# mjevans26/Satellite_ComputerVision

Measured on AMD Instinct MI355X. Metric: tiles/sec (train) 256x256x4 U-Net, higher is better.
Workload: dtype bf16; 1 GPU; U-Net 256x256x4 bfloat16 training, batch 64 per GPU (BASELINE configs[1]); global_batch=64, parallelism=dp1, loss=weighted_categorical_crossentropy, optimizer=adam(9e-4)

## Files before the change

satellite_computervision_amd/csrc/conv_bwd_fused.hip:

```cpp
#include "igemm_common.hpp"
#include <cstdlib>
#include <cstring>

#ifndef BWDF_ABL
#define BWDF_ABL 0
#endif
#define FABL(bit) ((BWDF_ABL & (bit)) != 0)

int wgrad_reduce_slabs(const float* ws, float* dw, int nslab, int taps, int kpad, int npad, int cin, int nvalid, int accumulate, hipStream_t st);
void reduce_job_fill(satcv_reduce_job* job, const float* ws, float* dw, int nslab, int taps, int kpad, int npad, int cin, int nvalid, int transposed, int accumulate);
void satcv_prof_begin(int kind, double flops, hipStream_t st);
void satcv_prof_end(int kind, hipStream_t st);

struct BwdfArgs {
  IgemmArgs e;
  const void* g; const void* yraw; int ldg;
  const float* bn_scale; const float* bn_shift; const float* bn_mean; const float* bn_rstd; const float* bn_coef; int bn_c, linear;
  const void* x0; const void* x1; int c0, c1;
  const float* in_scale; const float* in_shift; int in_relu;
  const void* w;
  float* ws;
  int tiles_x, tiles_y;
  satcv_stat_t* bst_sums; int bst_ld; const float* bst_mean; const float* bst_rstd;
  int bst_act_form;
  const void* dp; int lddp; const unsigned char* amax;
  const float* hg_dl; const float* hg_w;
};

__device__ __forceinline__ bf16x4 tr_read4(const bf16* p) {
  short4v v = __builtin_amdgcn_ds_read_tr16_b64_v4i16((__attribute__((address_space(3))) short4v*)(p));
  return __builtin_bit_cast(bf16x4, v);
}

template <int CIN, int COUT, int NW, int WPS, bool POOL = false, bool NODG = false, int CINS = CIN, bool HG = false>
__global__ __launch_bounds__(NW * 64, WPS) void bwd_fused_kernel(const BwdfArgs a, const int total_tiles) {
  static_assert(!HG || !POOL, "the head feeds a decoder block");
  typedef bf16 T;
  constexpr int TW = 32, TH = 8, BM = 256, RL = TH + 2, CL = TW + 2, PITCH = CL, EL = 8, NTHREADS = NW * 64;
  constexpr int SD = COUT / 8, SX = CIN / 8, SXR = CINS / 8;
  constexpr int DSTRIDE = RL * PITCH * EL;
  constexpr int XSTRIDE = BM * EL + 32;
  static_assert((DSTRIDE * 2) % 256 == 64 && (XSTRIDE * 2) % 256 == 64, "plane strides must be 64 B modulo 256 B");
  constexpr int D_ITEMS = RL * CL * SD, DI = (D_ITEMS + NTHREADS - 1) / NTHREADS;
  constexpr int X_ITEMS = BM * SXR, XI = X_ITEMS / NTHREADS;
  static_assert(X_ITEMS % NTHREADS == 0 && NTHREADS % SD == 0 && NTHREADS % SXR == 0, "item -> thread mapping");
  constexpr int XPIX_STEP = NTHREADS / SXR;
  static_assert(XPIX_STEP % 32 == 0, "x items of a thread must share a column");
  constexpr int MT = 8 / NW, NT = CIN / 32;
#ifdef BWDF_NOBAL
  constexpr int NTILE = (CIN / 32) * (COUT / 32) * 9, FULL = (NTILE + NW - 1) / NW, REM = 0, WT = FULL;
#else
  constexpr int NTILE = (CIN / 32) * (COUT / 32) * 9, FULL = NTILE / NW, REM = NTILE % NW, WT = FULL + (REM ? 1 : 0);
#endif
  constexpr bool GUARD = FULL * NW > NTILE;
  constexpr int WPP = REM ? NW / REM : 1, KPW = REM ? 16 / WPP : 0;
  static_assert(REM == 0 || (NW % REM == 0 && 16 % WPP == 0 && KPW % 2 == 0), "left-over products must split evenly along K");
  constexpr int W_ITEMS = NODG ? 0 : 9 * SD * CIN;
  constexpr size_t R0_BYTES = ((size_t)(SD * DSTRIDE + SX * XSTRIDE) * sizeof(T) + 127) / 128 * 128;
  constexpr size_t W_BYTES = (size_t)W_ITEMS * EL * sizeof(T);
  constexpr size_t O_BYTES = (size_t)BM * (CIN + 8) * sizeof(T);
  constexpr bool O_ALIAS = O_BYTES <= (size_t)SD * DSTRIDE * sizeof(T);
  constexpr size_t TAB_BYTES = (size_t)(SD * 32 + SX * 16 + (HG ? 2 * COUT : 0)) * sizeof(float);
  static_assert(!NODG || O_ALIAS || true, "");
  constexpr size_t O_OFF = O_ALIAS ? 0 : (R0_BYTES + W_BYTES + TAB_BYTES + 127) / 128 * 128;
  extern __shared__ __attribute__((aligned(16))) unsigned char smem_raw[];
  T* ldsD = reinterpret_cast<T*>(smem_raw);
  T* ldsX = ldsD + SD * DSTRIDE;
  T* ldsW = reinterpret_cast<T*>(smem_raw + R0_BYTES);
  float* tabD = reinterpret_cast<float*>(smem_raw + R0_BYTES + W_BYTES);
  float* tabX = tabD + SD * 32;
  float* tabH = tabX + SX * 16;

  const int tid = threadIdx.x, lane = tid & 63, wave = tid >> 6;
  const int r = lane & 31, hh = lane >> 5;
  const T* wp = reinterpret_cast<const T*>(a.w);

  for (int it = tid; it < W_ITEMS; it += NTHREADS) lstore8<T>(ldsW + (size_t)it * EL, gload8<T>(wp + (size_t)it * EL));
  if constexpr (SXR < SX) {
    for (int it = tid; it < (SX - SXR) * BM; it += NTHREADS) lstore8<T>(ldsX + (SXR + it / BM) * XSTRIDE + (it % BM) * EL, zero8<T>());
  }
  for (int ch = tid; ch < COUT; ch += NTHREADS) {
    const float sc = a.bn_scale[ch], sh = a.bn_shift[ch], mu = a.bn_mean[ch], rs = a.bn_rstd[ch], c1 = a.bn_coef[ch], c2 = a.bn_coef[a.bn_c + ch];
    float* t = tabD + (ch >> 3) * 32 + (ch & 7);
    t[0] = sc; t[8] = sh; t[16] = -sc * c2 * rs; t[24] = sc * (c2 * rs * mu - c1);
  }
  if constexpr (HG) {
    for (int ch = tid; ch < COUT; ch += NTHREADS) {
      float* t = tabH + (ch >> 3) * 16 + (ch & 7);
      t[0] = a.hg_w[ch * 2]; t[8] = a.hg_w[ch * 2 + 1];
    }
  }
  for (int ch = tid; ch < CINS; ch += NTHREADS) {
    float* t = tabX + (ch >> 3) * 16 + (ch & 7);
    t[0] = a.in_scale ? a.in_scale[ch] : 1.f; t[8] = a.in_scale ? a.in_shift[ch] : 0.f;
  }
  const float lin_lo = a.linear ? -INFINITY : 0.f;
  const bool xaff = a.in_scale != nullptr;
  const unsigned xrelu_lim = a.in_relu != 0 ? 0u : 0x80008000u;

  const int slot_d = tid % SD, slot_x = tid % SXR;
  constexpr int DPK = (DI + 2) / 3;
  unsigned d_pk[DPK];
#pragma unroll
  for (int k = 0; k < DPK; ++k) d_pk[k] = 0;
#pragma unroll
  for (int j = 0; j < DI; ++j) {
    const int it = tid + j * NTHREADS;
    const int p = it / SD, c = p % CL, L = p / CL;
    d_pk[j / 3] |= (unsigned)(it < D_ITEMS ? (L << 6) | c : 0x3ff) << (10 * (j % 3));
  }
  auto d_item = [&](int j) -> int { return (int)((d_pk[j / 3] >> (10 * (j % 3))) & 0x3ffu); };
  const int g_rowstride = a.e.w_ * a.ldg;
  const unsigned gy_lane = (unsigned)slot_d * EL;
  const int xch0 = slot_x * EL;
  const bool xsecond = xch0 >= a.c0;
  const T* xsrc = xsecond ? reinterpret_cast<const T*>(a.x1) + (xch0 - a.c0) : reinterpret_cast<const T*>(a.x0) + xch0;
  const int xcs = xsecond ? a.c1 : a.c0;
  const int xq0 = tid / SXR;
  const int x_l0 = slot_x * XSTRIDE + xq0 * EL;
  const int x_eoff0 = ((xq0 / TW) * a.e.w_ + (xq0 % TW)) * xcs, x_estep = (XPIX_STEP / TW) * a.e.w_ * xcs;

  int a_off[MT];
#pragma unroll
  for (int m = 0; m < MT; ++m) {
    const int q = (wave * MT + m) * 32 + r;
    a_off[m] = ((q / TW) * PITCH + (q % TW)) * EL;
  }
  const int gi = lane >> 4, i16 = lane & 15;
  const int chb = 16 * (gi & 1) + 4 * (i16 & 3);
  const int pk = 8 * (gi >> 1) + (i16 >> 2);
  const int tr_x = (chb >> 3) * XSTRIDE + pk * EL + (chb & 7);
  const int tr_d = (chb >> 3) * DSTRIDE + pk * EL + (chb & 7);

  auto tile_origin = [&](int v, int& n0, int& y0, int& x0) {
    const int tx = v % a.tiles_x; v /= a.tiles_x;
    const int ty = v % a.tiles_y;
    n0 = v / a.tiles_y; y0 = ty * TH; x0 = tx * TW;
  };
  auto next_origin = [&](int& n0, int& y0, int& x0) {
    x0 += TW;
    if (x0 >= a.e.w_) { x0 = 0; y0 += TH; if (y0 >= a.e.h) { y0 = 0; ++n0; } }
  };
  Raw8<T> rg[HG ? 1 : DI], ry[DI], rx[XI];
  float2 rdl[HG ? DI : 1];
  Raw8<T> rp[POOL ? DI : 1];
  uint2 ra[POOL ? DI : 1];
  const int hp = a.e.h >> 1, wpool = a.e.w_ >> 1;
  unsigned valid = 0;
  auto issue_loads = [&](int n0, int y0, int x0) -> unsigned {
    unsigned vm = 0;
    const int ylo = 1 - y0, yhi = a.e.h - y0 + 1, xlo = 1 - x0, xhi = a.e.w_ - x0 + 1;
    const long long pb = (long long)(n0 * a.e.h + y0 - 1) * a.e.w_ + (x0 - 1);
    const long long bp = pb * a.ldg;
    const T* gb = reinterpret_cast<const T*>(a.g) + bp;
    const T* yb = reinterpret_cast<const T*>(a.yraw) + bp;
    const unsigned centre = (unsigned)(g_rowstride + a.ldg) + gy_lane;
#pragma unroll
    for (int j = 0; j < DI; ++j) {
      const int pk_ = d_item(j), L = pk_ >> 6, c = pk_ & 63;
      const bool ok = pk_ != 0x3ff && L >= ylo && L < yhi && c >= xlo && c < xhi;
      vm |= (ok ? 1u : 0u) << j;
      unsigned off = ok ? (unsigned)(__mul24(L, g_rowstride) + __mul24(c, a.ldg)) + gy_lane : centre;
      asm volatile("" : "+v"(off));
      if constexpr (HG) {
        int poff = ok ? __mul24(L, a.e.w_) + c : a.e.w_ + 1;
        asm volatile("" : "+v"(poff));
        rdl[j] = reinterpret_cast<const float2*>(a.hg_dl)[pb + poff];
        ry[j] = gload8<T>(yb + off);
      } else if (!FABL(32)) { rg[j] = gload8<T>(gb + off); ry[j] = gload8<T>(yb + off); }
      else { rg[j] = zero8<T>(); ry[j] = zero8<T>(); rg[j].q[0].x = off; }
    }
    return vm;
  };
  auto issue_pool = [&](int n0, int y0, int x0) {
    if constexpr (POOL) {
      const int ylo = 1 - y0, yhi = a.e.h - y0 + 1, xlo = 1 - x0, xhi = a.e.w_ - x0 + 1;
      const size_t pb = (size_t)(n0 * hp + (y0 >> 1)) * wpool + (x0 >> 1);
#pragma unroll
      for (int j = 0; j < DI; ++j) {
        const int pk_ = d_item(j), L = pk_ >> 6, c = pk_ & 63;
        const bool ok = pk_ != 0x3ff && L >= ylo && L < yhi && c >= xlo && c < xhi;
        int po = ok ? __mul24((L - 1) >> 1, wpool) + ((c - 1) >> 1) : 0;
        asm volatile("" : "+v"(po));
        rp[j] = gload8<T>(reinterpret_cast<const T*>(a.dp) + (pb + po) * a.lddp + gy_lane);
        ra[j] = *reinterpret_cast<const uint2*>(a.amax + (pb + po) * COUT + gy_lane);
      }
    }
  };
  auto issue_x = [&](int n0, int y0, int x0) {
    const size_t bp = (size_t)(n0 * a.e.h + y0) * a.e.w_ + x0;
    const T* xb = xsrc + bp * xcs + x_eoff0;
#pragma unroll
    for (int j = 0; j < XI; ++j) { if (!FABL(32)) rx[j] = gload8<T>(xb + (size_t)j * x_estep); else { rx[j] = zero8<T>(); rx[j].q[0].x = (unsigned)(size_t)xb; } }
  };

  const int G = gridDim.x;
  const int xcd = blockIdx.x & 7, nx = G >> 3, remx = G & 7;
  const int bid = (xcd < remx ? xcd * (nx + 1) : remx * (nx + 1) + (xcd - remx) * nx) + (blockIdx.x >> 3);
  const int per = total_tiles / G, extra = total_tiles % G;
  const int t_lo = bid * per + (bid < extra ? bid : extra), t_hi = t_lo + per + (bid < extra ? 1 : 0);

  f32x16 wacc[WT];
  int w_xo[WT], w_do[WT];
#pragma unroll
  for (int t = 0; t < WT; ++t) {
#pragma unroll
    for (int i = 0; i < 16; ++i) wacc[t][i] = 0.f;
    const int wv = __builtin_amdgcn_readfirstlane(wave);
    const int id = t < FULL ? wv + t * NW : FULL * NW + wv / WPP;
    const int tap = id % 9, pair = id / 9;
    const int ci_t = pair % (CIN / 32), co_t = pair / (CIN / 32);
    w_xo[t] = ci_t * 4 * XSTRIDE;
    w_do[t] = co_t * 4 * DSTRIDE + ((2 - tap / 3) * PITCH + (2 - tap % 3)) * EL;
    if (t >= FULL) {
      const int k0 = (wv % WPP) * KPW;
      w_xo[t] += k0 * 16 * EL;
      w_do[t] += (k0 >> 1) * PITCH * EL;
    }
  }

  constexpr bool BST = !NODG && (WPS != 1 || POOL);
  float bs1[8], bs2[8];
#pragma unroll
  for (int e = 0; e < 8; ++e) { bs1[e] = 0.f; bs2[e] = 0.f; }
  int n0, y0, x0;
  if (t_lo < t_hi) { tile_origin(t_lo, n0, y0, x0); valid = issue_loads(n0, y0, x0); issue_x(n0, y0, x0); issue_pool(n0, y0, x0); }
  __syncthreads();
  for (int t = t_lo; t < t_hi; ++t) {
    {
      int toff = slot_d * 32;
      asm volatile("" : "+v"(toff));
      const float4* tp = reinterpret_cast<const float4*>(tabD + toff);
      float prm[32];
#pragma unroll
      for (int k = 0; k < 8; ++k) { const float4 v4 = tp[k]; prm[4 * k] = v4.x; prm[4 * k + 1] = v4.y; prm[4 * k + 2] = v4.z; prm[4 * k + 3] = v4.w; }
#pragma unroll
      for (int j = 0; j < DI; ++j) {
        float gv[8], yv[8];
        if constexpr (HG) {
          int hoff = slot_d * 16;
          asm volatile("" : "+v"(hoff));
          const float4* hp = reinterpret_cast<const float4*>(tabH + hoff);
          const float4 w00 = hp[0], w01 = hp[1], w10 = hp[2], w11 = hp[3];
          const float w0[8] = {w00.x, w00.y, w00.z, w00.w, w01.x, w01.y, w01.z, w01.w};
          const float w1[8] = {w10.x, w10.y, w10.z, w10.w, w11.x, w11.y, w11.z, w11.w};
#pragma unroll
          for (int e = 0; e < 8; ++e) gv[e] = (float)(T)fmaf(rdl[j].y, w1[e], rdl[j].x * w0[e]);
        } else {
          unpack8<T>(rg[j], gv);
        }
        unpack8<T>(ry[j], yv);
        if constexpr (POOL) {
          float pv[8];
          unpack8<T>(rp[j], pv);
          const int pk2 = d_item(j);
          const unsigned sub = ((((pk2 >> 6) + 1) & 1) << 1) | (((pk2 & 63) + 1) & 1);
#pragma unroll
          for (int e = 0; e < 8; ++e) {
            const unsigned am = ((e < 4 ? ra[j].x : ra[j].y) >> (8 * (e & 3))) & 0xffu;
            gv[e] += am == sub ? pv[e] : 0.f;
          }
        }
        Raw8<T> v;
        if constexpr (FABL(2) && !HG) { v = rg[j]; v.q[0].x ^= ry[j].q[0].x; }
        else {
          bf16x8 o;
#pragma unroll
          for (int e = 0; e < 8; ++e) {
            const float act = yv[e] * prm[e] + prm[8 + e];
            const float gm = act > lin_lo ? gv[e] : 0.f;
            o[e] = (bf16)(prm[e] * gm + (prm[16 + e] * yv[e] + prm[24 + e]));
          }
          v.q[0] = __builtin_bit_cast(uint4, o);
        }
        v = select8<T>((valid >> j) & 1u, v);
        const int pk_ = d_item(j);
        if (pk_ != 0x3ff) lstore8<T>(ldsD + slot_d * DSTRIDE + __mul24((pk_ >> 6) * CL + (pk_ & 63), EL), v);
        __builtin_amdgcn_sched_barrier(0);
      }
    }
    {
      float sc[8], sh[8];
      if (xaff) {
        int toff = slot_x * 16;
        asm volatile("" : "+v"(toff));
        const float4* tp = reinterpret_cast<const float4*>(tabX + toff);
        const float4 s0 = tp[0], s1 = tp[1], h0 = tp[2], h1 = tp[3];
        sc[0] = s0.x; sc[1] = s0.y; sc[2] = s0.z; sc[3] = s0.w; sc[4] = s1.x; sc[5] = s1.y; sc[6] = s1.z; sc[7] = s1.w;
        sh[0] = h0.x; sh[1] = h0.y; sh[2] = h0.z; sh[3] = h0.w; sh[4] = h1.x; sh[5] = h1.y; sh[6] = h1.z; sh[7] = h1.w;
      }
#pragma unroll
      for (int j = 0; j < XI; ++j) {
        Raw8<T> v = rx[j];
        if (xaff) v = affine8_lim(v, sc, sh, xrelu_lim);
        lstore8<T>(ldsX + x_l0 + j * (XPIX_STEP * EL), v);
      }
    }
    __syncthreads();
    const int tn0 = n0, ty0 = y0, tx0 = x0;
    if (t + 1 < t_hi) { next_origin(n0, y0, x0); valid = issue_loads(n0, y0, x0); }

#pragma unroll
    for (int tt = 0; tt < FULL; ++tt) {
      if (!FABL(8) && (!GUARD || tt < FULL - 1 || __builtin_amdgcn_readfirstlane(wave) + (FULL - 1) * NW < NTILE)) {
        const T* xa = ldsX + w_xo[tt] + tr_x;
        const T* da = ldsD + w_do[tt] + tr_d;
        bf16x4 fa[2][2], fb[2][2];
        auto read_k = [&](const T* xp, const T* dp, int u, int buf) {
          const int xq = u * 16 * EL, dq = ((u >> 1) * PITCH + (u & 1) * 16) * EL;
          fa[buf][0] = tr_read4(xp + xq); fa[buf][1] = tr_read4(xp + xq + 4 * EL);
          fb[buf][0] = tr_read4(dp + dq); fb[buf][1] = tr_read4(dp + dq + 4 * EL);
        };
        read_k(xa, da, 0, 0);
#pragma unroll 1
        for (int grp = 0; grp < TH / 2; ++grp) {
          const T* xp = xa + grp * (64 * EL);
          const T* dp = da + grp * (2 * PITCH * EL);
          const int wrap = grp + 1 < TH / 2 ? 1 : 1 - TH / 2;
#pragma unroll
          for (int u = 0; u < 4; ++u) {
            asm volatile("" ::: "memory");
            if (u < 3) read_k(xp, dp, u + 1, (u + 1) & 1);
            else read_k(xp + wrap * (64 * EL), dp + wrap * (2 * PITCH * EL), 0, 0);
            __builtin_amdgcn_sched_barrier(0);
            const bf16x8 afr = __builtin_shufflevector(fa[u & 1][0], fa[u & 1][1], 0, 1, 2, 3, 4, 5, 6, 7);
            const bf16x8 bfr = __builtin_shufflevector(fb[u & 1][0], fb[u & 1][1], 0, 1, 2, 3, 4, 5, 6, 7);
            if constexpr (!FABL(1)) wacc[tt] = __builtin_amdgcn_mfma_f32_32x32x16_bf16(afr, bfr, wacc[tt], 0, 0, 0);
            else asm volatile("" :: "v"(afr), "v"(bfr));
          }
        }
      }
    }
    if constexpr (REM > 0) {
      if (!FABL(8)) {
        const T* xa = ldsX + w_xo[FULL] + tr_x;
        const T* da = ldsD + w_do[FULL] + tr_d;
        bf16x4 fa[2][2], fb[2][2];
        auto read_k = [&](int u, int buf) {
          const int xq = u * 16 * EL, dq = ((u >> 1) * PITCH + (u & 1) * 16) * EL;
          fa[buf][0] = tr_read4(xa + xq); fa[buf][1] = tr_read4(xa + xq + 4 * EL);
          fb[buf][0] = tr_read4(da + dq); fb[buf][1] = tr_read4(da + dq + 4 * EL);
        };
        read_k(0, 0);
#pragma unroll
        for (int u = 0; u < KPW; ++u) {
          asm volatile("" ::: "memory");
          if (u + 1 < KPW) read_k(u + 1, (u + 1) & 1);
          __builtin_amdgcn_sched_barrier(0);
          const bf16x8 afr = __builtin_shufflevector(fa[u & 1][0], fa[u & 1][1], 0, 1, 2, 3, 4, 5, 6, 7);
          const bf16x8 bfr = __builtin_shufflevector(fb[u & 1][0], fb[u & 1][1], 0, 1, 2, 3, 4, 5, 6, 7);
          if constexpr (!FABL(1)) wacc[FULL] = __builtin_amdgcn_mfma_f32_32x32x16_bf16(afr, bfr, wacc[FULL], 0, 0, 0);
          else asm volatile("" :: "v"(afr), "v"(bfr));
        }
      }
    }
    if (t + 1 < t_hi) issue_x(n0, y0, x0);
    if (POOL && NODG && t + 1 < t_hi) issue_pool(n0, y0, x0);
    if constexpr (!NODG) {
    f32x16 acc[MT][NT];
#pragma unroll
    for (int m = 0; m < MT; ++m)
#pragma unroll
      for (int n = 0; n < NT; ++n)
#pragma unroll
        for (int i = 0; i < 16; ++i) acc[m][n][i] = 0.f;
    {
      constexpr int KS = COUT / 16, STEPS = 9 * KS;
      FragT<T> af[2][MT], bf[2][NT];
      auto read_step = [&](int st, int buf) {
        const int tap = st / KS, ks = st % KS;
        const int tap_off = ((tap / 3) * PITCH + (tap % 3)) * EL;
        const int slot = ks * 2 + hh;
#pragma unroll
        for (int m = 0; m < MT; ++m) af[buf][m] = lds_frag<T>(ldsD + slot * DSTRIDE + a_off[m] + tap_off);
#pragma unroll
        for (int n = 0; n < NT; ++n) bf[buf][n] = lds_frag<T>(ldsW + ((tap * SD + slot) * CIN + n * 32 + r) * EL);
      };
      if constexpr (!FABL(8)) {
      read_step(0, 0);
#pragma unroll
      for (int st = 0; st < STEPS; ++st) {
        asm volatile("" ::: "memory");
        if (st + 1 < STEPS) read_step(st + 1, (st + 1) & 1);
        __builtin_amdgcn_sched_barrier(0);
#pragma unroll
        for (int m = 0; m < MT; ++m)
#pragma unroll
          for (int n = 0; n < NT; ++n) {
            if constexpr (!FABL(1)) mma32<T>(acc[m][n], af[st & 1][m], bf[st & 1][n]);
            else asm volatile("" :: "v"(af[st & 1][m].v), "v"(bf[st & 1][n].v));
          }
      }
      }
    }
    if (POOL && t + 1 < t_hi) issue_pool(n0, y0, x0);
    __syncthreads();
    {
      constexpr int OPITCH = CIN + 8, VPR = CIN / 8;
      T* ldsO = reinterpret_cast<T*>(smem_raw + O_OFF);
      T* op = ldsO + ((wave * MT) * 32 + 4 * hh) * OPITCH + r;
#pragma unroll
      for (int m = 0; m < MT; ++m)
#pragma unroll
        for (int n = 0; n < NT; ++n)
#pragma unroll
          for (int i = 0; i < 16; ++i) op[(m * 32 + (i & 3) + 8 * (i >> 2)) * OPITCH + n * 32] = (T)acc[m][n][i];
      __syncthreads();
      const int vq = tid % VPR;
      T* yp = reinterpret_cast<T*>(a.e.y) + ((size_t)(tn0 * a.e.h + ty0) * a.e.w_ + tx0) * a.e.ldy + vq * 8;
      const unsigned row_pitch = (unsigned)a.e.w_ * a.e.ldy;
      const T* xact = ldsX + vq * XSTRIDE;
#pragma unroll 2
      for (int it = tid; it < BM * VPR; it += NTHREADS) {
        const int q = it / VPR;
        const uint4 dv = *reinterpret_cast<const uint4*>(ldsO + q * OPITCH + vq * 8);
        if constexpr (!FABL(4)) *reinterpret_cast<uint4*>(yp + (size_t)((q / TW) * row_pitch + (q % TW) * (unsigned)a.e.ldy)) = dv;
        else asm volatile("" :: "v"(dv.x));
        if (BST && a.bst_sums) {
          const bf16x8 d8 = __builtin_bit_cast(bf16x8, dv);
          const bf16x8 a8 = *reinterpret_cast<const bf16x8*>(xact + q * EL);
#pragma unroll
          for (int e = 0; e < 8; ++e) {
            const float df = (float)d8[e], af = (float)a8[e];
            bs1[e] += af > 0.f ? df : 0.f;
            bs2[e] += df * af;
          }
        }
      }
    }
    }
    __syncthreads();
  }
  if constexpr (REM > 0) {
    float* red = reinterpret_cast<float*>(smem_raw);
#pragma unroll
    for (int i = 0; i < 16; ++i) red[(wave * 16 + i) * 64 + lane] = wacc[FULL][i];
    __syncthreads();
    if (wave % WPP == 0) {
#pragma unroll 1
      for (int k = 1; k < WPP; ++k)
#pragma unroll
        for (int i = 0; i < 16; ++i) wacc[FULL][i] += red[((wave + k) * 16 + i) * 64 + lane];
    }
  }
#pragma unroll
  for (int tt = 0; tt < WT; ++tt) {
    const int wv = __builtin_amdgcn_readfirstlane(wave);
    const int id = tt < FULL ? wv + tt * NW : FULL * NW + wv / WPP;
    if ((tt < FULL && (!GUARD || id < NTILE)) || (tt >= FULL && wv % WPP == 0)) {
      const int tap = id % 9, pair = id / 9;
      const int ci_t = pair % (CIN / 32), co_t = pair / (CIN / 32);
      float* dst = a.ws + ((size_t)(blockIdx.x * 9 + tap) * CIN + ci_t * 32) * COUT + co_t * 32 + r;
#pragma unroll
      for (int i = 0; i < 16; ++i) dst[(size_t)((i & 3) + 8 * (i >> 2) + 4 * hh) * COUT] = wacc[tt][i];
    }
  }
  if (BST && a.bst_sums && t_lo < t_hi) {
    constexpr int VPR = CIN / 8, NPER = NTHREADS / VPR;
    float* red = reinterpret_cast<float*>(smem_raw);
    __syncthreads();
#pragma unroll
    for (int e = 0; e < 8; ++e) { red[e * NTHREADS + tid] = bs1[e]; red[(8 + e) * NTHREADS + tid] = bs2[e]; }
    __syncthreads();
    if (tid < CIN) {
      const int vq = tid >> 3, e = tid & 7;
      double t1 = 0.0, t2 = 0.0;
      for (int k = 0; k < NPER; ++k) { t1 += (double)red[e * NTHREADS + k * VPR + vq]; t2 += (double)red[(8 + e) * NTHREADS + k * VPR + vq]; }
      double s2 = t2;
      if (!a.bst_act_form) {
        const double sc = (double)a.in_scale[tid], sh = (double)a.in_shift[tid], mu = (double)a.bst_mean[tid], rs = (double)a.bst_rstd[tid];
        s2 = sc != 0.0 ? (t2 - (sh + sc * mu) * t1) * (rs / sc) : 0.0;
      }
      satcv_stat_t* rowp = a.bst_sums + (size_t)(blockIdx.x % SATCV_STAT_ROWS) * 2 * a.bst_ld;
      atomicAdd(rowp + tid, (satcv_stat_t)t1);
      atomicAdd(rowp + a.bst_ld + tid, (satcv_stat_t)s2);
    }
  }
}

template <int CIN, int COUT, int NW, bool NODG = false>
struct BwdfGeom {
  static constexpr int SD = COUT / 8, SX = CIN / 8;
  static constexpr size_t R0 = ((size_t)(SD * (10 * 34 * 8) + SX * (256 * 8 + 32)) * 2 + 127) / 128 * 128;
  static constexpr size_t O_BYTES = (size_t)256 * (CIN + 8) * 2;
  static constexpr bool O_ALIAS = O_BYTES <= (size_t)SD * (10 * 34 * 8) * 2;
  static constexpr size_t BASE = R0 + (NODG ? 0 : (size_t)9 * SD * CIN * 16) + (size_t)(SD * 32 + SX * 16 + 2 * COUT) * 4;
  static constexpr size_t LDS0 = O_ALIAS ? BASE : (BASE + 127) / 128 * 128 + O_BYTES;
  static constexpr size_t RED = (size_t)16 * NW * 64 * 4;
  static constexpr size_t LDS = LDS0 > RED ? LDS0 : RED;
};

static int g_ncu = 0;
static int bwdf_grid(size_t lds, int waves, int wps, long long total) {
  if (!g_ncu) {
    int dev = 0; hipDeviceProp_t p;
    if (hipGetDevice(&dev) != hipSuccess || hipGetDeviceProperties(&p, dev) != hipSuccess) return -1;
    g_ncu = p.multiProcessorCount;
  }
  int per_cu = (int)((160 * 1024) / lds);
  const int by_waves = 4 * wps / waves;
  if (per_cu > by_waves) per_cu = by_waves;
  if (per_cu < 1) per_cu = 1;
  long long grid = (long long)g_ncu * per_cu;
  if (grid > total) grid = total;
  return (int)grid;
}

static bool bwdf_shape_ok(const satcv_bwdf_desc* d, int& cin_s) {
  cin_s = d->c0 + d->c1;
  if (d->dtype != SATCV_BF16 || d->kh != 3 || d->kw != 3 || d->dil != 1) return false;
  if (d->x1 && d->c0 % 8 != 0) return false;
  if (d->h % 8 != 0 || d->w_ % 32 != 0) return false;
  if (d->ldg % 8 != 0 || ((uintptr_t)d->g % 16) != 0 || ((uintptr_t)d->yraw % 16) != 0) return false;
  if (d->hg_dlogits && (!d->hg_w || d->hg_ncls != 2 || d->dpool || ((uintptr_t)d->hg_dlogits % 8) != 0)) return false;
  if (d->dx && (d->lddx % 8 != 0 || ((uintptr_t)d->dx % 16) != 0)) return false;
  if ((long long)d->w_ * d->ldg >= (1 << 23)) return false;
  if (d->dpool) {
    if (!d->amax || d->lddp % 8 != 0 || ((uintptr_t)d->dpool % 16) != 0 || ((uintptr_t)d->amax % 8) != 0 || d->x1) return false;
    if (d->dx) return cin_s == 32 && d->cin == 32 && d->cout == 64;
    return cin_s == 16 && d->cin <= 16 && d->cout == 32 && !d->bst_sums;
  }
  if (!d->dx) return false;
  if (d->bst_sums && cin_s == 64 && d->cout == 64) return false;
  if (!((cin_s == 32 && d->cout == 32) || (cin_s == 64 && d->cout == 32) || (cin_s == 64 && d->cout == 64))) return false;
  if (d->cin != cin_s) return false;
  return true;
}

template <int CIN, int COUT, int NW, int WPS, bool POOL = false, bool NODG = false, int CINS = CIN, bool HG = false>
static int bwdf_launch(const satcv_bwdf_desc* d, hipStream_t st, bool query, int64_t* ws_bytes, satcv_reduce_job* job = nullptr) {
  using G = BwdfGeom<CIN, COUT, NW, NODG>;
  static_assert(G::LDS <= 160 * 1024, "tile + weights exceed the LDS");
  const long long total = (long long)d->n * (d->h / 8) * (d->w_ / 32);
  const int grid = bwdf_grid(G::LDS, NW, WPS, total);
  if (grid <= 0) { satcv_set_error("bwd_fused: device query failed"); return SATCV_ERR_HIP; }
  const size_t need = (size_t)grid * 9 * CIN * COUT * sizeof(float);
  if (job) { reduce_job_fill(job, d->workspace, d->dw, grid, 9, CIN, COUT, d->cin, COUT, 0, d->accumulate); return SATCV_OK; }
  if (query) { *ws_bytes = (int64_t)need; return SATCV_OK; }
  SATCV_CHECK((size_t)d->workspace_bytes >= need, "bwd_fused: workspace %lld < %zu", (long long)d->workspace_bytes, need);
  BwdfArgs a;
  memset(&a, 0, sizeof(a));
  a.e.y = d->dx; a.e.ldy = d->lddx; a.e.n = d->n; a.e.h = d->h; a.e.w_ = d->w_; a.e.cout = CIN; a.e.cout_pad = CIN; a.e.cstat = CIN;
  a.e.imgs = 1; a.e.rpi = 8; a.e.tiles_x = d->w_ / 32; a.e.tiles_y = d->h / 8; a.e.n_tiles = 1;
  a.g = d->g; a.yraw = d->yraw; a.ldg = d->ldg;
  a.bn_scale = d->bn_scale; a.bn_shift = d->bn_shift; a.bn_mean = d->bn_mean; a.bn_rstd = d->bn_rstd; a.bn_coef = d->bn_coef; a.bn_c = d->cout; a.linear = d->linear;
  a.x0 = d->x0; a.x1 = d->x1; a.c0 = d->c0; a.c1 = d->c1; a.in_scale = d->in_scale; a.in_shift = d->in_shift; a.in_relu = d->in_relu;
  a.w = d->w_dgrad; a.ws = d->workspace; a.tiles_x = d->w_ / 32; a.tiles_y = d->h / 8;
  a.bst_sums = d->bst_sums; a.bst_ld = d->bst_sums_ld; a.bst_mean = d->bst_mean; a.bst_rstd = d->bst_rstd; a.bst_act_form = d->bst_act_form;
  a.dp = d->dpool; a.lddp = d->lddp; a.amax = reinterpret_cast<const unsigned char*>(d->amax);
  a.hg_dl = d->hg_dlogits; a.hg_w = d->hg_w;
  auto kern = bwd_fused_kernel<CIN, COUT, NW, WPS, POOL, NODG, CINS, HG>;
  { const int rc = satcv_ensure_dynamic_lds(reinterpret_cast<const void*>(kern), G::LDS); if (rc) return rc; }
  const double flops = (NODG ? 2.0 : 4.0) * d->n * d->h * d->w_ * (double)CINS * COUT * 9;
  satcv_prof_begin(3, flops, st);
  hipLaunchKernelGGL(kern, dim3(grid), dim3(NW * 64), G::LDS, st, a, (int)total);
  satcv_prof_end(3, st);
  hipError_t e = hipGetLastError();
  if (e != hipSuccess) { satcv_set_error("bwd_fused launch: %s", hipGetErrorString(e)); return SATCV_ERR_HIP; }
  if (d->defer_reduce) return SATCV_OK;
  return wgrad_reduce_slabs(d->workspace, d->dw, grid, 9, CIN, COUT, d->cin, COUT, d->accumulate, st);
}

static int bwdf_dispatch(const satcv_bwdf_desc* d, hipStream_t st, bool query, int64_t* ws_bytes, satcv_reduce_job* job = nullptr) {
  int cin_s;
  if (!bwdf_shape_ok(d, cin_s)) return SATCV_ERR_UNSUPPORTED;
  if (d->dpool) {
    if (d->dx) return bwdf_launch<32, 64, 4, 1, true, false>(d, st, query, ws_bytes, job);
    return bwdf_launch<32, 32, 8, 2, true, true, 16>(d, st, query, ws_bytes, job);
  }
  if (cin_s == 32 && d->hg_dlogits) return bwdf_launch<32, 32, 8, 2, false, false, 32, true>(d, st, query, ws_bytes, job);
  if (d->hg_dlogits) return SATCV_ERR_UNSUPPORTED;
  if (cin_s == 32) return bwdf_launch<32, 32, 8, 2>(d, st, query, ws_bytes, job);
  if (d->cout == 32) return bwdf_launch<64, 32, 8, 2>(d, st, query, ws_bytes, job);
  return bwdf_launch<64, 64, 4, 1>(d, st, query, ws_bytes, job);
}

extern "C" int satcv_conv2d_bwd_fused_reduce_job(const satcv_bwdf_desc* d, satcv_reduce_job* job) {
  SATCV_CHECK(d && job && d->dw && d->workspace, "bwd_fused_reduce_job: null pointer");
  return bwdf_dispatch(d, nullptr, false, nullptr, job);
}

extern "C" int64_t satcv_conv2d_bwd_fused_workspace(const satcv_bwdf_desc* d) {
  int64_t nb = -1;
  if (!d || bwdf_dispatch(d, nullptr, true, &nb) != SATCV_OK) return -1;
  return nb;
}

extern "C" int satcv_conv2d_bwd_fused(const satcv_bwdf_desc* d, void* stream) {
  SATCV_CHECK(d && (d->g || d->hg_dlogits) && d->yraw && d->x0 && d->dw && d->workspace && (d->dx == nullptr || d->w_dgrad), "bwd_fused: null pointer");
  SATCV_CHECK(d->bn_scale && d->bn_shift && d->bn_mean && d->bn_rstd && d->bn_coef, "bwd_fused: BatchNorm coefficients missing");
  SATCV_CHECK((d->c1 == 0) == (d->x1 == nullptr) && d->n > 0 && d->h > 0 && d->w_ > 0, "bwd_fused: bad dims");
  SATCV_CHECK(!d->bst_sums || (d->bst_sums_ld >= d->c0 + d->c1 && (d->bst_act_form ? d->in_scale == nullptr
                               : (d->in_scale && d->in_shift && d->in_relu && d->bst_mean && d->bst_rstd))),
              "bwd_fused: the fused sums need the input's BatchNorm (in_scale / in_shift with ReLU, bst_mean / bst_rstd), or an activated input with bst_act_form");
  const int rc = bwdf_dispatch(d, reinterpret_cast<hipStream_t>(stream), false, nullptr);
  if (rc == SATCV_ERR_UNSUPPORTED) satcv_set_error("bwd_fused: shape outside the kernel's limits (ask satcv_conv2d_bwd_fused_workspace first)");
  return rc;
}
```

Measured before the change: 8362 tiles/s.

## Assign wgrad waves per channel-tile pair, sharing X fragments across taps

Reworks how the fused backward kernel splits weight-gradient MFMA work across waves. Work used to be distributed as independent (tap, ci-tile, co-tile) products. Each wave now owns one (ci, co) tile pair, a group of taps and a share of K. It reads each X fragment once from LDS and reuses it across several tap accumulators, which cuts LDS read traffic for X. Partial K sums are then reduced through LDS with extra barriers. For the 64x32 case the X staging is also moved ahead of the D staging. The cost is more accumulator registers per wave and added synchronization in the reduction epilogue.

```diff
diff --git a/satellite_computervision_amd/csrc/conv_bwd_fused.hip b/satellite_computervision_amd/csrc/conv_bwd_fused.hip
--- a/satellite_computervision_amd/csrc/conv_bwd_fused.hip
+++ b/satellite_computervision_amd/csrc/conv_bwd_fused.hip
@@ -47,14 +47,11 @@
   constexpr int XPIX_STEP = NTHREADS / SXR;
   static_assert(XPIX_STEP % 32 == 0, "x items of a thread must share a column");
   constexpr int MT = 8 / NW, NT = CIN / 32;
-#ifdef BWDF_NOBAL
-  constexpr int NTILE = (CIN / 32) * (COUT / 32) * 9, FULL = (NTILE + NW - 1) / NW, REM = 0, WT = FULL;
-#else
-  constexpr int NTILE = (CIN / 32) * (COUT / 32) * 9, FULL = NTILE / NW, REM = NTILE % NW, WT = FULL + (REM ? 1 : 0);
-#endif
-  constexpr bool GUARD = FULL * NW > NTILE;
-  constexpr int WPP = REM ? NW / REM : 1, KPW = REM ? 16 / WPP : 0;
-  static_assert(REM == 0 || (NW % REM == 0 && 16 % WPP == 0 && KPW % 2 == 0), "left-over products must split evenly along K");
+  constexpr int NPAIR = (CIN / 32) * (COUT / 32), RW = NW / NPAIR;
+  static_assert(NW % NPAIR == 0 && (RW == 1 || RW == 2 || RW == 4 || RW == 8), "waves per (ci-tile, co-tile) pair");
+  constexpr int TG = (RW >= 4 || (POOL && RW == 2)) ? 2 : 1, KSP = RW / TG, NTP = (9 + TG - 1) / TG, KN = 16 / KSP, NG = KN / 4;
+  static_assert(KN % 4 == 0, "a K share is whole groups of four k-steps (two tile rows)");
+  constexpr bool XFIRST = CIN == 64 && COUT == 32;
   constexpr int W_ITEMS = NODG ? 0 : 9 * SD * CIN;
   constexpr size_t R0_BYTES = ((size_t)(SD * DSTRIDE + SX * XSTRIDE) * sizeof(T) + 127) / 128 * 128;
   constexpr size_t W_BYTES = (size_t)W_ITEMS * EL * sizeof(T);
@@ -200,23 +197,21 @@
   const int per = total_tiles / G, extra = total_tiles % G;
   const int t_lo = bid * per + (bid < extra ? bid : extra), t_hi = t_lo + per + (bid < extra ? 1 : 0);
 
-  f32x16 wacc[WT];
-  int w_xo[WT], w_do[WT];
-#pragma unroll
-  for (int t = 0; t < WT; ++t) {
-#pragma unroll
-    for (int i = 0; i < 16; ++i) wacc[t][i] = 0.f;
-    const int wv = __builtin_amdgcn_readfirstlane(wave);
-    const int id = t < FULL ? wv + t * NW : FULL * NW + wv / WPP;
-    const int tap = id % 9, pair = id / 9;
-    const int ci_t = pair % (CIN / 32), co_t = pair / (CIN / 32);
-    w_xo[t] = ci_t * 4 * XSTRIDE;
-    w_do[t] = co_t * 4 * DSTRIDE + ((2 - tap / 3) * PITCH + (2 - tap % 3)) * EL;
-    if (t >= FULL) {
-      const int k0 = (wv % WPP) * KPW;
-      w_xo[t] += k0 * 16 * EL;
-      w_do[t] += (k0 >> 1) * PITCH * EL;
-    }
+  const int wv = __builtin_amdgcn_readfirstlane(wave);
+  const int w_ks = wv % KSP, w_tg = TG == 1 ? 0 : (wv / KSP) % TG, w_pair = wv / (KSP * TG);
+  const int w_ci = w_pair % (CIN / 32), w_co = w_pair / (CIN / 32);
+  const int w_tap0 = w_tg * NTP;
+  const int w_xo = w_ci * 4 * XSTRIDE + w_ks * KN * 16 * EL;
+  const int w_do = w_co * 4 * DSTRIDE + ((w_ks * KN) >> 1) * PITCH * EL;
+  const bool w_last = w_tap0 + NTP <= 9;
+  f32x16 wacc[NTP];
+  int w_to[NTP];
+#pragma unroll
+  for (int j = 0; j < NTP; ++j) {
+#pragma unroll
+    for (int i = 0; i < 16; ++i) wacc[j][i] = 0.f;
+    const int tap = w_tap0 + j < 9 ? w_tap0 + j : 8;
+    w_to[j] = ((2 - tap / 3) * PITCH + (2 - tap % 3)) * EL;
   }
 
   constexpr bool BST = !NODG && (WPS != 1 || POOL);
@@ -227,6 +222,24 @@
   if (t_lo < t_hi) { tile_origin(t_lo, n0, y0, x0); valid = issue_loads(n0, y0, x0); issue_x(n0, y0, x0); issue_pool(n0, y0, x0); }
   __syncthreads();
   for (int t = t_lo; t < t_hi; ++t) {
+    auto stage_x = [&]() {
+      float sc[8], sh[8];
+      if (xaff) {
+        int toff = slot_x * 16;
+        asm volatile("" : "+v"(toff));
+        const float4* tp = reinterpret_cast<const float4*>(tabX + toff);
+        const float4 s0 = tp[0], s1 = tp[1], h0 = tp[2], h1 = tp[3];
+        sc[0] = s0.x; sc[1] = s0.y; sc[2] = s0.z; sc[3] = s0.w; sc[4] = s1.x; sc[5] = s1.y; sc[6] = s1.z; sc[7] = s1.w;
+        sh[0] = h0.x; sh[1] = h0.y; sh[2] = h0.z; sh[3] = h0.w; sh[4] = h1.x; sh[5] = h1.y; sh[6] = h1.z; sh[7] = h1.w;
+      }
+#pragma unroll
+      for (int j = 0; j < XI; ++j) {
+        Raw8<T> v = rx[j];
+        if (xaff) v = affine8_lim(v, sc, sh, xrelu_lim);
+        lstore8<T>(ldsX + x_l0 + j * (XPIX_STEP * EL), v);
+      }
+    };
+    if constexpr (XFIRST) stage_x();
     {
       int toff = slot_d * 32;
       asm volatile("" : "+v"(toff));
@@ -279,78 +292,51 @@
         __builtin_amdgcn_sched_barrier(0);
       }
     }
-    {
-      float sc[8], sh[8];
-      if (xaff) {
-        int toff = slot_x * 16;
-        asm volatile("" : "+v"(toff));
-        const float4* tp = reinterpret_cast<const float4*>(tabX + toff);
-        const float4 s0 = tp[0], s1 = tp[1], h0 = tp[2], h1 = tp[3];
-        sc[0] = s0.x; sc[1] = s0.y; sc[2] = s0.z; sc[3] = s0.w; sc[4] = s1.x; sc[5] = s1.y; sc[6] = s1.z; sc[7] = s1.w;
-        sh[0] = h0.x; sh[1] = h0.y; sh[2] = h0.z; sh[3] = h0.w; sh[4] = h1.x; sh[5] = h1.y; sh[6] = h1.z; sh[7] = h1.w;
-      }
-#pragma unroll
-      for (int j = 0; j < XI; ++j) {
-        Raw8<T> v = rx[j];
-        if (xaff) v = affine8_lim(v, sc, sh, xrelu_lim);
-        lstore8<T>(ldsX + x_l0 + j * (XPIX_STEP * EL), v);
-      }
-    }
+    if constexpr (!XFIRST) stage_x();
     __syncthreads();
     const int tn0 = n0, ty0 = y0, tx0 = x0;
     if (t + 1 < t_hi) { next_origin(n0, y0, x0); valid = issue_loads(n0, y0, x0); }
 
-#pragma unroll
-    for (int tt = 0; tt < FULL; ++tt) {
-      if (!FABL(8) && (!GUARD || tt < FULL - 1 || __builtin_amdgcn_readfirstlane(wave) + (FULL - 1) * NW < NTILE)) {
-        const T* xa = ldsX + w_xo[tt] + tr_x;
-        const T* da = ldsD + w_do[tt] + tr_d;
-        bf16x4 fa[2][2], fb[2][2];
-        auto read_k = [&](const T* xp, const T* dp, int u, int buf) {
-          const int xq = u * 16 * EL, dq = ((u >> 1) * PITCH + (u & 1) * 16) * EL;
-          fa[buf][0] = tr_read4(xp + xq); fa[buf][1] = tr_read4(xp + xq + 4 * EL);
-          fb[buf][0] = tr_read4(dp + dq); fb[buf][1] = tr_read4(dp + dq + 4 * EL);
-        };
-        read_k(xa, da, 0, 0);
+    if (!FABL(8)) {
+      const T* xa = ldsX + w_xo + tr_x;
+      const T* da = ldsD + w_do + tr_d;
+      bf16x4 fa[2][2], fb[NTP][2];
+      auto read_x = [&](const T* xp, int u, int buf) {
+        const int xq = u * 16 * EL;
+        fa[buf][0] = tr_read4(xp + xq); fa[buf][1] = tr_read4(xp + xq + 4 * EL);
+      };
+      auto read_d = [&](const T* dp, int u, int j) {
+        const T* p = dp + ((u >> 1) * PITCH + (u & 1) * 16) * EL + w_to[j];
+        fb[j][0] = tr_read4(p); fb[j][1] = tr_read4(p + 4 * EL);
+      };
+      read_x(xa, 0, 0);
+#pragma unroll
+      for (int j = 0; j < NTP; ++j) if (j < NTP - 1 || w_last) read_d(da, 0, j);
 #pragma unroll 1
-        for (int grp = 0; grp < TH / 2; ++grp) {
-          const T* xp = xa + grp * (64 * EL);
-          const T* dp = da + grp * (2 * PITCH * EL);
-          const int wrap = grp + 1 < TH / 2 ? 1 : 1 - TH / 2;
-#pragma unroll
-          for (int u = 0; u < 4; ++u) {
-            asm volatile("" ::: "memory");
-            if (u < 3) read_k(xp, dp, u + 1, (u + 1) & 1);
-            else read_k(xp + wrap * (64 * EL), dp + wrap * (2 * PITCH * EL), 0, 0);
-            __builtin_amdgcn_sched_barrier(0);
-            const bf16x8 afr = __builtin_shufflevector(fa[u & 1][0], fa[u & 1][1], 0, 1, 2, 3, 4, 5, 6, 7);
-            const bf16x8 bfr = __builtin_shufflevector(fb[u & 1][0], fb[u & 1][1], 0, 1, 2, 3, 4, 5, 6, 7);
-            if constexpr (!FABL(1)) wacc[tt] = __builtin_amdgcn_mfma_f32_32x32x16_bf16(afr, bfr, wacc[tt], 0, 0, 0);
-            else asm volatile("" :: "v"(afr), "v"(bfr));
-          }
-        }
-      }
-    }
-    if constexpr (REM > 0) {
-      if (!FABL(8)) {
-        const T* xa = ldsX + w_xo[FULL] + tr_x;
-        const T* da = ldsD + w_do[FULL] + tr_d;
-        bf16x4 fa[2][2], fb[2][2];
-        auto read_k = [&](int u, int buf) {
-          const int xq = u * 16 * EL, dq = ((u >> 1) * PITCH + (u & 1) * 16) * EL;
-          fa[buf][0] = tr_read4(xa + xq); fa[buf][1] = tr_read4(xa + xq + 4 * EL);
-          fb[buf][0] = tr_read4(da + dq); fb[buf][1] = tr_read4(da + dq + 4 * EL);
-        };
-        read_k(0, 0);
-#pragma unroll
-        for (int u = 0; u < KPW; ++u) {
+      for (int grp = 0; grp < NG; ++grp) {
+        const T* xp = xa + grp * (64 * EL);
+        const T* dp = da + grp * (2 * PITCH * EL);
+        const int wrap = grp + 1 < NG ? 1 : 1 - NG;
+#pragma unroll
+        for (int u = 0; u < 4; ++u) {
+          const T* xn = u < 3 ? xp : xp + wrap * (64 * EL);
+          const T* dn = u < 3 ? dp : dp + wrap * (2 * PITCH * EL);
+          const int un = u < 3 ? u + 1 : 0;
           asm volatile("" ::: "memory");
-          if (u + 1 < KPW) read_k(u + 1, (u + 1) & 1);
+          read_x(xn, un, (u + 1) & 1);
           __builtin_amdgcn_sched_barrier(0);
           const bf16x8 afr = __builtin_shufflevector(fa[u & 1][0], fa[u & 1][1], 0, 1, 2, 3, 4, 5, 6, 7);
-          const bf16x8 bfr = __builtin_shufflevector(fb[u & 1][0], fb[u & 1][1], 0, 1, 2, 3, 4, 5, 6, 7);
-          if constexpr (!FABL(1)) wacc[FULL] = __builtin_amdgcn_mfma_f32_32x32x16_bf16(afr, bfr, wacc[FULL], 0, 0, 0);
-          else asm volatile("" :: "v"(afr), "v"(bfr));
+#pragma unroll
+          for (int j = 0; j < NTP; ++j) {
+            if (j < NTP - 1 || w_last) {
+              const bf16x8 bfr = __builtin_shufflevector(fb[j][0], fb[j][1], 0, 1, 2, 3, 4, 5, 6, 7);
+              if constexpr (!FABL(1)) wacc[j] = __builtin_amdgcn_mfma_f32_32x32x16_bf16(afr, bfr, wacc[j], 0, 0, 0);
+              else asm volatile("" :: "v"(afr), "v"(bfr));
+              __builtin_amdgcn_sched_barrier(0);
+              read_d(dn, un, j);
+              __builtin_amdgcn_sched_barrier(0);
+            }
+          }
         }
       }
     }
@@ -431,28 +417,32 @@
     }
     __syncthreads();
   }
-  if constexpr (REM > 0) {
+  if constexpr (KSP > 1) {
     float* red = reinterpret_cast<float*>(smem_raw);
 #pragma unroll
-    for (int i = 0; i < 16; ++i) red[(wave * 16 + i) * 64 + lane] = wacc[FULL][i];
-    __syncthreads();
-    if (wave % WPP == 0) {
+    for (int j = 0; j < NTP; ++j) {
+      if (w_ks != 0) {
+#pragma unroll
+        for (int i = 0; i < 16; ++i) red[(wave * 16 + i) * 64 + lane] = wacc[j][i];
+      }
+      __syncthreads();
+      if (w_ks == 0) {
 #pragma unroll 1
-      for (int k = 1; k < WPP; ++k)
-#pragma unroll
-        for (int i = 0; i < 16; ++i) wacc[FULL][i] += red[((wave + k) * 16 + i) * 64 + lane];
-    }
-  }
-#pragma unroll
-  for (int tt = 0; tt < WT; ++tt) {
-    const int wv = __builtin_amdgcn_readfirstlane(wave);
-    const int id = tt < FULL ? wv + tt * NW : FULL * NW + wv / WPP;
-    if ((tt < FULL && (!GUARD || id < NTILE)) || (tt >= FULL && wv % WPP == 0)) {
-      const int tap = id % 9, pair = id / 9;
-      const int ci_t = pair % (CIN / 32), co_t = pair / (CIN / 32);
-      float* dst = a.ws + ((size_t)(blockIdx.x * 9 + tap) * CIN + ci_t * 32) * COUT + co_t * 32 + r;
-#pragma unroll
-      for (int i = 0; i < 16; ++i) dst[(size_t)((i & 3) + 8 * (i >> 2) + 4 * hh) * COUT] = wacc[tt][i];
+        for (int k = 1; k < KSP; ++k)
+#pragma unroll
+          for (int i = 0; i < 16; ++i) wacc[j][i] += red[((wave + k) * 16 + i) * 64 + lane];
+      }
+      __syncthreads();
+    }
+  }
+  if (w_ks == 0) {
+#pragma unroll
+    for (int j = 0; j < NTP; ++j) {
+      if (w_tap0 + j < 9) {
+        float* dst = a.ws + ((size_t)(blockIdx.x * 9 + w_tap0 + j) * CIN + w_ci * 32) * COUT + w_co * 32 + r;
+#pragma unroll
+        for (int i = 0; i < 16; ++i) dst[(size_t)((i & 3) + 8 * (i >> 2) + 4 * hh) * COUT] = wacc[j][i];
+      }
     }
   }
   if (BST && a.bst_sums && t_lo < t_hi) {
```

After: 8361 tiles/s, median of 2. No clear change (-0.0%).
